# PeterFWS/Structure-PLP-SLAM

Hardware: AMD Instinct MI355X
Metric: frames/sec ORB+LSD extract+match, 640x480 TUM-RGBD, 1/2/4/8 GPU (higher is better)
Workload: dtype u8

## Files before the change

### structure-plp-slam_amd/csrc/match_kernels.hip

```cpp
#include <hip/hip_runtime.h>
#include <stdint.h>
#include <cstdlib>

#include "libstdcxx_sort.hpp"
#include "plp_barrier.hpp"
#include "match_device.hpp"
#include "plp_common.hpp"
#include "xcd_map.hpp"

namespace plp {

__device__ __forceinline__ int floor_d(double v) { int i = (int)v; return i - (i > v); }
__device__ __forceinline__ int ceil_d(double v) { int i = (int)v; return i + (i < v); }

__device__ __forceinline__ unsigned hamming256(const uint4& a0, const uint4& a1, const uint4& b0, const uint4& b1) {
    return __popc(a0.x ^ b0.x) + __popc(a0.y ^ b0.y) + __popc(a0.z ^ b0.z) + __popc(a0.w ^ b0.w) +
           __popc(a1.x ^ b1.x) + __popc(a1.y ^ b1.y) + __popc(a1.z ^ b1.z) + __popc(a1.w ^ b1.w);
}

__device__ __forceinline__ unsigned long long wave_min_u64(unsigned long long v) {
#pragma unroll
    for (int o = 32; o > 0; o >>= 1) {
        const unsigned lo = __shfl_xor((unsigned)v, o), hi = __shfl_xor((unsigned)(v >> 32), o);
        const unsigned long long w = ((unsigned long long)hi << 32) | lo;
// ... 326 lines not shown
                auto bc_f = [&](float v) -> float { return __int_as_float(__builtin_amdgcn_readlane(__float_as_int(v), u)); };
                LineTarget T;
                T.sx = bc_f(f_sx); T.sy = bc_f(f_sy); T.ex = bc_f(f_ex); T.ey = bc_f(f_ey); T.xr = bc_f(f_xr); T.xr2 = bc_f(f_xr2);
                const int misc = __builtin_amdgcn_readlane(f_misc, u);
                T.octave = misc >> 8; T.occ = (misc >> 4) & 1; T.kp_oct = (unsigned)misc & 15u;
                if (!active || !line_gate<FAM>(P, c, T, t_xr != nullptr)) continue;
                const int t = base + u;
                const uint4* d = reinterpret_cast<const uint4*>(t_desc + 32 * (size_t)t);
                const unsigned dist = hamming256(q0, q1, d[0], d[1]);
                ++passed;
                topk_insert(top, ((unsigned long long)dist << 32) | ((unsigned long long)(unsigned)t << 4) | T.kp_oct);
            }
        }
    } else if (!(c.windowed && c.empty))
        for (int t = 0; t < n; ++t) {
            const unsigned long long key = candidate_key<FAM>(P, c, t, kps, t_desc, t_xr, t_occ, q0, q1);
            if (key == ~0ull) continue;
            ++passed;
            topk_insert(top, key);
        }
    if (!active) return;
#pragma unroll
    for (int r = 0; r < kMatchK; ++r) klist[r] = pack_key(top[r]);
    *kcount = passed;
}
template <int FAM>
__global__ __launch_bounds__(64) void k_match_topk_lanes(MatchProblem P) {
    const int b = blockIdx.y;
    const int m = P.q_counts ? min(P.q_counts[b], P.m_cap) : P.m_cap;
    for (int qblock = blockIdx.x; qblock * 64 < m; qblock += gridDim.x) match_topk_lanes_block<FAM>(P, b, qblock, m);
}

constexpr int kQueriesPerBlock = 128;
constexpr int kCellStride = 4104;

__global__ __launch_bounds__(256) void k_match_prep(MatchProblem P) {
    __shared__ uint32_t cnt2[2048];
    __shared__ uint16_t start[4098];
    __shared__ uint16_t tmp_t[8192];
    __shared__ int part[4];
    const int tid = threadIdx.x, b = blockIdx.x;
    const int n = P.t_counts ? min(P.t_counts[b], P.n_cap) : P.n_cap;
    const int ncell = P.grid_cols * P.grid_rows;
    const plp_keypoint* kps = P.t_kps + (size_t)b * P.n_cap;
    const float* t_xr = P.t_x_right ? P.t_x_right + (size_t)b * P.n_cap : nullptr;
    const uint8_t* t_occ = P.t_occupied ? P.t_occupied + (size_t)b * P.n_cap : nullptr;
    StagedTarget* st = P.sorted + (size_t)b * P.n_cap;
    float* sxr = P.sorted_xr + (size_t)b * P.n_cap;
    auto cnt_inc = [&](int c) -> int { return (int)((atomicAdd(&cnt2[c >> 1], 1u << (16 * (c & 1))) >> (16 * (c & 1))) & 0xffffu); };
    for (int i = tid; i < 2048; i += 256) cnt2[i] = 0;
    wg_barrier();
    auto cell_xy = [&](float x, float y, bool occ, int& cx, int& cy) -> bool {
        cx = floor_d((double)__fsub_rn(x, P.grid_min_x) * P.inv_cell_w);
        cy = floor_d((double)__fsub_rn(y, P.grid_min_y) * P.inv_cell_h);
        return cx >= 0 && cx < P.grid_cols && cy >= 0 && cy < P.grid_rows && !occ;
    };
    for (int t0 = tid; t0 < n; t0 += 4 * 256) {
        float kx[4], ky[4]; bool oc[4];
#pragma unroll
        for (int u = 0; u < 4; ++u) { const int t = min(t0 + 256 * u, n - 1); kx[u] = kps[t].x; ky[u] = kps[t].y; oc[u] = t_occ && t_occ[t]; }
#pragma unroll
        for (int u = 0; u < 4; ++u) {
            int cx, cy;
            if (t0 + 256 * u < n && cell_xy(kx[u], ky[u], oc[u], cx, cy)) cnt_inc(cx * P.grid_rows + cy);
        }
    }
    wg_barrier();
    {
        const int lane = tid & 63, wv = tid >> 6;
        int c16[16], sum = 0;
#pragma unroll
        for (int i = 0; i < 8; ++i) { const uint32_t w = cnt2[tid * 8 + i]; c16[2 * i] = (int)(w & 0xffffu); c16[2 * i + 1] = (int)(w >> 16); sum += c16[2 * i] + c16[2 * i + 1]; }
        int inc = sum;
#pragma unroll
        for (int o = 1; o < 64; o <<= 1) { const int up = __shfl_up(inc, o); if (lane >= o) inc += up; }
        if (lane == 63) part[wv] = inc;
        wg_barrier();
        int base = inc - sum;
        for (int k = 0; k < wv; ++k) base += part[k];
#pragma unroll
        for (int i = 0; i < 16; ++i) { start[tid * 16 + i] = (uint16_t)base; base += c16[i]; }
        if (tid == 255) { start[4096] = (uint16_t)base; start[4097] = (uint16_t)base; }
        wg_barrier();
        for (int i = tid; i < 2048; i += 256) cnt2[i] = 0;
        wg_barrier();
    }
    for (int t0 = tid; t0 < n; t0 += 4 * 256) {
        float kx[4], ky[4]; bool oc[4];
#pragma unroll
        for (int u = 0; u < 4; ++u) { const int t = min(t0 + 256 * u, n - 1); kx[u] = kps[t].x; ky[u] = kps[t].y; oc[u] = t_occ && t_occ[t]; }
#pragma unroll
        for (int u = 0; u < 4; ++u) {
            const int t = t0 + 256 * u;
            int cx, cy;
            if (t >= n || !cell_xy(kx[u], ky[u], oc[u], cx, cy)) continue;
            const int cell = cx * P.grid_rows + cy;
            tmp_t[start[cell] + cnt_inc(cell)] = (uint16_t)t;
        }
    }
    wg_barrier();
    const int used = start[4096];
    for (int p0 = tid; p0 < used; p0 += 4 * 256) {
        int tt[4]; float kx[4], ky[4], xr[4] = {0.f, 0.f, 0.f, 0.f}; int ko[4];
#pragma unroll
        for (int u = 0; u < 4; ++u) {
            tt[u] = tmp_t[min(p0 + 256 * u, used - 1)];
            kx[u] = kps[tt[u]].x; ky[u] = kps[tt[u]].y; ko[u] = kps[tt[u]].octave;
            if (t_xr) xr[u] = t_xr[tt[u]];
        }
#pragma unroll
        for (int u = 0; u < 4; ++u) {
            if (p0 + 256 * u >= used) continue;
            const int t = tt[u];
            int cx, cy;
            cell_xy(kx[u], ky[u], false, cx, cy);
            const int cell = cx * P.grid_rows + cy, s0 = start[cell], s1 = start[cell + 1];
            int rank = 0;
            for (int j = s0; j < s1; ++j) rank += (int)tmp_t[j] < t;
            StagedTarget r;
            r.x = kx[u]; r.y = ky[u]; r.packed = ((uint32_t)ko[u] & 0xffu) | ((uint32_t)cx << 8) | ((uint32_t)cy << 16); r.t = (uint32_t)t;
            st[s0 + rank] = r;
            if (t_xr) sxr[s0 + rank] = xr[u];
        }
    }
    for (int i = tid; i <= ncell; i += 256) P.cell_start[(size_t)b * kCellStride + i] = start[min(i, 4096)];
}

constexpr int kLanePend = 8;
#define PLP_TOPK_CELLS_BOUNDS __launch_bounds__(256) __attribute__((amdgpu_waves_per_eu(6, 8)))

__device__ __forceinline__ uint32_t row16_min_u32(uint32_t v) {
    v = min(v, (uint32_t)__builtin_amdgcn_update_dpp((int)v, (int)v, 0x128, 0xf, 0xf, false));
    v = min(v, (uint32_t)__builtin_amdgcn_update_dpp((int)v, (int)v, 0x124, 0xf, 0xf, false));
    v = min(v, (uint32_t)__builtin_amdgcn_update_dpp((int)v, (int)v, 0x122, 0xf, 0xf, false));
    v = min(v, (uint32_t)__builtin_amdgcn_update_dpp((int)v, (int)v, 0x121, 0xf, 0xf, false));
    return v;
}
__device__ __forceinline__ int row16_sum_i32(int v) {
    v += __builtin_amdgcn_update_dpp(v, v, 0x128, 0xf, 0xf, false);
    v += __builtin_amdgcn_update_dpp(v, v, 0x124, 0xf, 0xf, false);
    v += __builtin_amdgcn_update_dpp(v, v, 0x122, 0xf, 0xf, false);
    v += __builtin_amdgcn_update_dpp(v, v, 0x121, 0xf, 0xf, false);
    return v;
}

__global__ PLP_TOPK_CELLS_BOUNDS void k_match_topk_cells(MatchProblem P, int qpb) {
    extern __shared__ __attribute__((aligned(16))) uint8_t smem[];
    unsigned uqb, ub;
    xcd_frame_major(uqb, ub);
    const int tid = threadIdx.x, b = (int)ub;
    const int m = P.q_counts ? min(P.q_counts[b], P.m_cap) : P.m_cap;
    const int q_begin = (int)uqb * qpb;
    if (q_begin >= m) return;
    const int ncell = P.grid_cols * P.grid_rows, rows = P.grid_rows;
    const uint8_t* t_desc = P.t_desc + (size_t)b * P.n_cap * 32;
    const bool has_xr = P.t_x_right != nullptr;
    const int nb = P.lds_targets;
    float2* sxy = reinterpret_cast<float2*>(smem);
    uint32_t* sto = reinterpret_cast<uint32_t*>(smem + (size_t)nb * 8);
    float* sxr = reinterpret_cast<float*>(smem + (size_t)nb * 12);
    uint16_t* cs = reinterpret_cast<uint16_t*>(smem + (size_t)nb * (has_xr ? 16 : 12));
    const uint4* g_sorted = reinterpret_cast<const uint4*>(P.sorted + (size_t)b * P.n_cap);
    const float* g_sorted_xr = P.sorted_xr + (size_t)b * P.n_cap;
    {
        const uint16_t* gcs = P.cell_start + (size_t)b * kCellStride;
        const int used = min((int)gcs[ncell], nb);
        for (int i0 = tid; i0 < used; i0 += 4 * 256) {
            uint4 r[4]; float xr[4] = {0.f, 0.f, 0.f, 0.f};
#pragma unroll
            for (int u = 0; u < 4; ++u) { const int i = min(i0 + 256 * u, used - 1); r[u] = g_sorted[i]; if (has_xr) xr[u] = g_sorted_xr[i]; }
#pragma unroll
            for (int u = 0; u < 4; ++u) {
                const int i = i0 + 256 * u;
                if (i < used) {
                    sxy[i] = make_float2(__uint_as_float(r[u].x), __uint_as_float(r[u].y));
                    sto[i] = (r[u].w & 0xffffu) | ((r[u].z & 0xffu) << 16);
                    if (has_xr) sxr[i] = xr[u];
                }
            }
        }
        const uint32_t* g32 = reinterpret_cast<const uint32_t*>(gcs);
        for (int i = tid; i < (ncell + 2) / 2; i += 256) reinterpret_cast<uint32_t*>(cs)[i] = g32[i];
    }
    __shared__ int s_dir;
    if (tid == 0) s_dir = query_direction(P, b);
    wg_barrier();
    typedef const __attribute__((address_space(3))) uint32_t* lds_u32; typedef const __attribute__((address_space(3))) float* lds_f32;
    const lds_f32 sxy_l = (lds_f32)sxy; const lds_u32 sto_l = (lds_u32)sto; const lds_f32 sxr_l = (lds_f32)sxr;
    auto t_xy = [&](int i) -> float2 { if (i < nb) return make_float2(sxy_l[2 * i], sxy_l[2 * i + 1]); const uint4 r = g_sorted[i]; return make_float2(__uint_as_float(r.x), __uint_as_float(r.y)); };
    auto t_to = [&](int i) -> uint32_t { if (i < nb) return sto_l[i]; const uint4 r = g_sorted[i]; return (r.w & 0xffffu) | ((r.z & 0xffu) << 16); };
    auto t_xr = [&](int i) -> float { return i < nb ? sxr_l[i] : g_sorted_xr[i]; };
    const uint8_t* q_valid = P.q_valid ? P.q_valid + (size_t)b * P.m_cap : nullptr;
    const int q_end = min(m, q_begin + qpb);
    static_assert(kLanePend % 2 == 0, "two positions per register");
    const int lane = tid & 63, wv = __builtin_amdgcn_readfirstlane(tid >> 6);
    for (int q_wave = q_begin + 64 * wv; q_wave < q_end; q_wave += 256) {
        const int q = q_wave + lane;
        const bool in_range = q < q_end;
        const bool active = in_range && !(q_valid && !q_valid[q]);
        uint32_t top[kMatchK], ovf[kMatchK];
#pragma unroll
        for (int i = 0; i < kMatchK; ++i) { top[i] = 0xffffffffu; ovf[i] = 0xffffffffu; }
        auto insert = [&](uint32_t key) {
            if (key < top[kMatchK - 1]) {
                const uint32_t out = top[kMatchK - 1];
                top[kMatchK - 1] = key;
#pragma unroll
                for (int e = kMatchK - 1; e > 0; --e) { const uint32_t lo = min(top[e], top[e - 1]), hi = max(top[e], top[e - 1]); top[e - 1] = lo; top[e] = hi; }
                key = out;
            }
            if (key < ovf[kMatchK - 1]) {
                ovf[kMatchK - 1] = key;
#pragma unroll
                for (int e = kMatchK - 1; e > 0; --e) { const uint32_t lo = min(ovf[e], ovf[e - 1]), hi = max(ovf[e], ovf[e - 1]); ovf[e - 1] = lo; ovf[e] = hi; }
            }
        };
        int passed = 0;
        float rx = 0.f, ry = 0.f, mg = 0.f, qxr = 0.f;
        uint32_t win = 1u, lvls = 255u << 16;
        int i = 0, i1 = 0;
        uint4 q0 = make_uint4(0u, 0u, 0u, 0u), q1 = q0;
        if (active) {
            const QueryCtx c = make_query(P, q, b, s_dir);
            if (!c.empty) {
                const uint4* qd = reinterpret_cast<const uint4*>(P.q_desc + ((size_t)b * P.q_desc_stride + q) * 32);
                q0 = qd[0]; q1 = qd[1];
                rx = c.rx; ry = c.ry; mg = c.mg; qxr = c.xr;
                win = (uint32_t)c.min_cx | ((uint32_t)c.max_cx << 8) | ((uint32_t)c.min_cy << 16) | ((uint32_t)c.max_cy << 24);
                lvls = (uint32_t)min(max(c.min_level, 0), 256) | ((c.max_level < 0 ? 255u : (uint32_t)min(c.max_level, 255)) << 16);
            }
        }
        bool wave_more;
        do {
            uint32_t pend[kLanePend / 2];
#pragma unroll
            for (int k = 0; k < kLanePend / 2; ++k) pend[k] = 0u;
            int nc = 0;
            for (;;) {
                if (i >= i1) {
                    const int col = (int)(win & 0xffu);
                    if (col <= (int)((win >> 8) & 0xffu)) {
                        i = cs[col * rows + (int)((win >> 16) & 0xffu)]; i1 = cs[col * rows + (int)(win >> 24) + 1];
                        ++win;
                    }
                } else {
                    const int p = i++;
                    const float2 sp = t_xy(p);
                    const uint32_t oct = t_to(p) >> 16;
                    bool ok = (lvls & 0xffffu) <= oct && oct <= (lvls >> 16) && fabsf(__fsub_rn(sp.x, rx)) < mg && fabsf(__fsub_rn(sp.y, ry)) < mg;
                    if (ok && has_xr) {
                        const float xr = t_xr(p);
                        ok = !(0 < xr && mg < fabsf(__fsub_rn(qxr, xr)));
                    }
                    if (ok) {
                        const uint32_t v = (uint32_t)p << (16 * (nc & 1));
#pragma unroll
                        for (int k = 0; k < kLanePend / 2; ++k) pend[k] |= (nc >> 1) == k ? v : 0u;
                        ++nc;
                    }
                }
                wave_more = __builtin_amdgcn_ballot_w64(i < i1 || (win & 0xffu) <= ((win >> 8) & 0xffu)) != 0ull;
                if (!wave_more || __builtin_amdgcn_ballot_w64(nc == kLanePend) != 0ull) break;
            }
            auto slot_pos = [&](int j) -> int { return (int)((pend[j >> 1] >> (16 * (j & 1))) & 0xffffu); };
            auto gather = [&](int j, uint4& a0, uint4& a1) {
                if (j < nc) {
                    const uint4* d = reinterpret_cast<const uint4*>(t_desc + 32 * (size_t)(t_to(slot_pos(j)) & 0xffffu));
                    a0 = d[0]; a1 = d[1];
                }
            };
            uint4 a0 = make_uint4(0u, 0u, 0u, 0u), a1 = a0;
            gather(0, a0, a1);
#pragma unroll
            for (int j = 0; j < kLanePend; ++j) {
                if (__builtin_amdgcn_ballot_w64(j < nc) == 0ull) break;
                uint4 b0 = a0, b1 = a1;
                if (j + 1 < kLanePend) gather(j + 1, b0, b1);
                if (j < nc) insert((hamming256(q0, q1, a0, a1) << 16) | (uint32_t)slot_pos(j));
                a0 = b0; a1 = b1;
            }
            passed += nc;
        } while (wave_more);
        if (!in_range) continue;
        uint32_t e[kMatchK];
#pragma unroll
        for (int k = 0; k < kMatchK; ++k) {
            e[k] = 0xffffffffu;
            if (top[k] != 0xffffffffu) {
                const uint32_t to = t_to((int)(top[k] & 0xffffu));
                e[k] = ((top[k] >> 16) << 20) | (((to >> 16) & 15u) << 16) | (to & 0xffffu);
            }
        }
        static_assert(kMatchK == 8, "two 16-byte stores per query");
        uint4* out = reinterpret_cast<uint4*>(P.klist + ((size_t)b * P.m_cap + q) * kMatchK);
        out[0] = make_uint4(e[0], e[1], e[2], e[3]);
        out[1] = make_uint4(e[4], e[5], e[6], e[7]);
        P.kcount[(size_t)b * P.m_cap + q] = active ? passed : -1;
        if (passed > kMatchK) {
#pragma unroll
            for (int k = 0; k < kMatchK; ++k) {
                e[k] = 0xffffffffu;
                if (ovf[k] != 0xffffffffu) {
                    const uint32_t to = t_to((int)(ovf[k] & 0xffffu));
                    e[k] = ((ovf[k] >> 16) << 20) | (((to >> 16) & 15u) << 16) | (to & 0xffffu);
                }
            }
            uint4* out2 = reinterpret_cast<uint4*>(P.klist2 + ((size_t)b * P.m_cap + q) * kMatchK);
            out2[0] = make_uint4(e[0], e[1], e[2], e[3]);
            out2[1] = make_uint4(e[4], e[5], e[6], e[7]);
        }
    }
}

__global__ __launch_bounds__(256) void k_match_topk_lds(MatchProblem P) {
    extern __shared__ __attribute__((aligned(16))) uint8_t smem[];
    const int tid = threadIdx.x, lane = tid & 63, wv = __builtin_amdgcn_readfirstlane(tid >> 6), b = blockIdx.y;
    const int m = P.q_counts ? min(P.q_counts[b], P.m_cap) : P.m_cap;
    const int q_begin = blockIdx.x * kQueriesPerBlock;
    if (q_begin >= m) return;
    const int n = P.t_counts ? min(P.t_counts[b], P.n_cap) : P.n_cap;
    const uint8_t* t_desc = P.t_desc + (size_t)b * P.n_cap * 32;
    uint4* sdesc = reinterpret_cast<uint4*>(smem);
    {
        const uint4* src = reinterpret_cast<const uint4*>(t_desc);
        for (int i = tid; i < 2 * n; i += 256) sdesc[i] = src[i];
    }
    wg_barrier();
    const uint8_t* q_valid = P.q_valid ? P.q_valid + (size_t)b * P.m_cap : nullptr;
    for (int q = q_begin + wv; q < min(m, q_begin + kQueriesPerBlock); q += 4) {
        uint32_t* klist = P.klist + ((size_t)b * P.m_cap + q) * kMatchK;
        int32_t* kcount = P.kcount + (size_t)b * P.m_cap + q;
        if (q_valid && !q_valid[q]) { if (lane == 0) *kcount = -1; continue; }
        const uint4* qd = reinterpret_cast<const uint4*>(P.q_desc + ((size_t)b * P.q_desc_stride + q) * 32);
        const uint4 q0 = qd[0], q1 = qd[1];
        unsigned long long top[kMatchK];
#pragma unroll
        for (int i = 0; i < kMatchK; ++i) top[i] = ~0ull;
        int passed = 0;
        for (int t = lane; t < n; t += 64) {
            const unsigned dist = hamming256(q0, q1, sdesc[2 * t], sdesc[2 * t + 1]);
            ++passed;
            topk_insert(top, ((unsigned long long)dist << 32) | ((unsigned long long)(unsigned)t << 4));
        }
#pragma unroll
        for (int o = 32; o > 0; o >>= 1) passed += __shfl_xor(passed, o);
        topk_merge_store(top, lane, klist);
        if (lane == 0) *kcount = passed;
    }
}

template <int FAM = kFamAny>
__device__ __forceinline__ bool accept(const MatchProblem& P, unsigned best, int best_lvl, unsigned second, int second_lvl) {
    const int mode = fam_mode<FAM>(P.mode);
    if (mode == PLP_MATCH_MODE_LANDMARKS || mode == PLP_MATCH_MODE_LANDMARKS_LINE) {
        if (!(best <= 100u)) return false;
        if (best_lvl == second_lvl && (float)best > __fmul_rn(P.lowe_ratio, (float)second)) return false;
        return true;
    }
    if (is_last_frame_mode(mode)) return best <= (P.hamm_dist_thr > 0 ? (unsigned)P.hamm_dist_thr : 100u);
    if (mode == PLP_MATCH_MODE_TRIANGULATION) return true;
    if (50u < best) return false;
    if (__fmul_rn(P.lowe_ratio, (float)second) < (float)best) return false;
    return true;
}

template <bool kSorted, int FAM = kFamAny>
__device__ __forceinline__ void match_resolve_body(const MatchProblem& P) {
    const int mode = fam_mode<FAM>(P.mode);
    extern __shared__ int32_t lds[];
    __shared__ int s_changed, s_num, s_hist[32], s_valid_bin[32], s_full_n, s_claim_tmp[256], s_sort_ws[48];
    __shared__ unsigned s_sort_idx[32];
    __shared__ int s_dir;
    const int tid = threadIdx.x, lane = tid & 63, wv = __builtin_amdgcn_readfirstlane(tid >> 6), b = blockIdx.x;
    const int m = P.q_counts ? min(P.q_counts[b], P.m_cap) : P.m_cap;
    const int n = P.t_counts ? min(P.t_counts[b], P.n_cap) : P.n_cap;
    int32_t* owner_final = lds;
    int32_t* owner_prev = lds + P.n_cap;
    int32_t* owner_next = lds + 2 * P.n_cap;
    const uint32_t* klist = P.klist + (size_t)b * P.m_cap * kMatchK;
    const int32_t* kcount = P.kcount + (size_t)b * P.m_cap;
    int32_t* claim = P.claim + (size_t)b * P.m_cap;
    const uint8_t* has_obs = P.q_has_obs ? P.q_has_obs + (size_t)b * P.m_cap : nullptr;
    const plp_keypoint* kps = P.t_kps ? P.t_kps + (size_t)b * P.n_cap : nullptr;
    const uint8_t* t_desc = P.t_desc + (size_t)b * P.n_cap * 32;
    const float* t_xr = P.t_x_right ? P.t_x_right + (size_t)b * P.n_cap : nullptr;
    const uint8_t* t_occ = P.t_occupied ? P.t_occupied + (size_t)b * P.n_cap : nullptr;
    int32_t* out = P.out_match + (size_t)b * P.n_cap;

    for (int t = tid; t < n; t += 256) { owner_final[t] = 0x7fffffff; out[t] = -1; }
    for (int q = tid; q < m; q += 256) claim[q] = -1;
    if (is_last_frame_mode(mode) && tid == 0) s_dir = query_direction(P, b);
    wg_barrier();

    int32_t* full_list = P.full_list + (size_t)b * P.m_cap;
    const int need = (is_last_frame_mode(mode) || mode == PLP_MATCH_MODE_TRIANGULATION) ? 1 : 2;
    const bool blocks_always = !has_obs || mode == PLP_MATCH_MODE_BRUTE_FORCE || is_group_mode(mode);
    const unsigned t_flip = mode == PLP_MATCH_MODE_TRIANGULATION ? 0xffffu : 0u;
    constexpr bool use_sorted = kSorted;
    const StagedTarget* sorted = P.sorted + (size_t)b * P.n_cap;
    const float* sorted_xr = P.sorted_xr + (size_t)b * P.n_cap;
    const uint16_t* g_cell_start = P.cell_start + (size_t)b * kCellStride;
    auto taken = [&](int t, int q, int) -> bool { return owner_final[t] != 0x7fffffff || owner_prev[t] < q; };
    {
        for (int chunk_start = 0; chunk_start < m; chunk_start += 256) {
          const int q = chunk_start + tid;
          int my_claim = -1;
          for (int t = tid; t < n; t += 256) owner_prev[t] = 0x7fffffff;
          constexpr int kList = kSorted ? 2 * kMatchK : kMatchK;
          uint32_t e8[kList];
          int cnt = 0;
          if (q < m) {
              cnt = kcount[q];
              const uint4* kp = reinterpret_cast<const uint4*>(klist + (size_t)q * kMatchK);
              const uint4 lo = kp[0], hi = kp[1];
              e8[0] = lo.x; e8[1] = lo.y; e8[2] = lo.z; e8[3] = lo.w; e8[4] = hi.x; e8[5] = hi.y; e8[6] = hi.z; e8[7] = hi.w;
              if constexpr (kSorted) {
#pragma unroll
                  for (int k = kMatchK; k < kList; ++k) e8[k] = 0xffffffffu;
                  if (cnt > kMatchK) {
                      const uint4* kp2 = reinterpret_cast<const uint4*>(P.klist2 + ((size_t)b * P.m_cap + q) * kMatchK);
                      const uint4 lo2 = kp2[0], hi2 = kp2[1];
                      e8[8] = lo2.x; e8[9] = lo2.y; e8[10] = lo2.z; e8[11] = lo2.w; e8[12] = hi2.x; e8[13] = hi2.y; e8[14] = hi2.z; e8[15] = hi2.w;
                  }
              }
          }
          for (int inner = 0; inner <= 256; ++inner) {
            if (tid == 0) { s_full_n = 0; s_changed = 0; }
            for (int t = tid; t < n; t += 256) owner_next[t] = 0x7fffffff;
            wg_barrier();
            int new_claim = -1;
            bool decided = false;
            if (q < m) {
                if (cnt <= 0) decided = true;
                else {
                    const int have = min(cnt, kList);
                    unsigned best = 256, second = 256;
                    int best_lvl = -1, second_lvl = -1, best_t = -1, found = 0;
#pragma unroll
                    for (int e = 0; e < kList; ++e) {
                        if (e >= have || found >= need) continue;
                        const int t = (int)((e8[e] & 0xffff) ^ t_flip);
                        if (taken(t, q, chunk_start)) continue;
                        if (found == 0) { best = e8[e] >> 20; best_lvl = (int)((e8[e] >> 16) & 15); best_t = t; }
                        else { second = e8[e] >> 20; second_lvl = (int)((e8[e] >> 16) & 15); }
                        ++found;
                    }
                    bool rescan = found < need && cnt > kList;
                    if (rescan && mode != PLP_MATCH_MODE_TRIANGULATION) {
                        const unsigned d8 = e8[kList - 1] >> 20;
                        const bool lm = mode == PLP_MATCH_MODE_LANDMARKS || mode == PLP_MATCH_MODE_LANDMARKS_LINE;
                        const unsigned thr = (lm || is_last_frame_mode(mode)) ? (is_last_frame_mode(mode) && P.hamm_dist_thr > 0 ? (unsigned)P.hamm_dist_thr : 100u) : 50u;
                        if (found == 0) { if (d8 > thr) rescan = false; }
                        else if (best > thr) rescan = false;
                        else if (lm) { if (!((float)best > __fmul_rn(P.lowe_ratio, (float)d8))) { rescan = false; second = d8; second_lvl = -2; } }
                        else if (!(__fmul_rn(P.lowe_ratio, (float)d8) < (float)best)) { rescan = false; second = d8; }
                    }
                    if (rescan) full_list[atomicAdd(&s_full_n, 1)] = q;
                    else { decided = true; if (found > 0 && accept<FAM>(P, best, best_lvl, second, second_lvl)) new_claim = best_t; }
                }
            }
            wg_barrier();
            const int nf = s_full_n;
            if (tid == 0 && P.dbg && nf) atomicAdd(&P.dbg[0], nf);
            for (int f = wv; f < nf; f += 4) {
                const int fq = full_list[f];
                const QueryCtx c = make_query<FAM>(P, fq, b, s_dir);
                const uint4* qd = reinterpret_cast<const uint4*>(P.q_desc + ((size_t)b * P.q_desc_stride + fq) * 32);
                const uint4 q0 = qd[0], q1 = qd[1];
                unsigned long long k0 = ~0ull, k1 = ~0ull;
                if constexpr (use_sorted) {
                    if (!c.empty) {
                        const bool check_level = (0 < c.min_level) || (0 <= c.max_level);
                        for (int col = c.min_cx; col <= c.max_cx; ++col) {
                            const int i0 = g_cell_start[col * P.grid_rows + c.min_cy], i1 = g_cell_start[col * P.grid_rows + c.max_cy + 1];
                            for (int i = i0 + lane; i < i1; i += 64) {
                                const StagedTarget s = sorted[i];
                                const int oct = (int)(s.packed & 0xff);
                                if (check_level) {
                                    if (oct < c.min_level) continue;
                                    if (0 <= c.max_level && c.max_level < oct) continue;
                                }
                                if (!(fabsf(__fsub_rn(s.x, c.rx)) < c.mg && fabsf(__fsub_rn(s.y, c.ry)) < c.mg)) continue;
                                if (t_xr) {
                                    const float xr = sorted_xr[i];
                                    if (0 < xr && c.mg < fabsf(__fsub_rn(c.xr, xr))) continue;
                                }
                                if (taken((int)s.t, fq, chunk_start)) continue;
                                const uint4* d = reinterpret_cast<const uint4*>(t_desc + 32 * (size_t)s.t);
                                const unsigned dist = hamming256(q0, q1, d[0], d[1]);
                                const unsigned long long key = ((unsigned long long)dist << 32) | ((unsigned long long)(unsigned)i << 4) | (unsigned)(oct & 15);
                                if (key < k0) { k1 = k0; k0 = key; } else if (key < k1) k1 = key;
                            }
                        }
                    }
                } else if (!(c.windowed && c.empty)) {
                    for (int t = lane; t < n; t += 64) {
                        if (taken(t, fq, chunk_start)) continue;
                        const unsigned long long key = candidate_key<FAM>(P, c, t, kps, t_desc, t_xr, t_occ, q0, q1);
                        if (key < k0) { k1 = k0; k0 = key; } else if (key < k1) k1 = key;
                    }
                }
                const unsigned long long g0 = wave_min_u64(k0);
                const unsigned long long g1 = wave_min_u64(k0 == g0 ? k1 : k0);
                if (lane == 0) {
                    int nc = -1;
                    if (g0 != ~0ull) {
                        const unsigned second = g1 != ~0ull ? (unsigned)(g1 >> 32) : 256u;
                        const int second_lvl = g1 != ~0ull ? (int)(g1 & 15) : -1;
                        if (accept<FAM>(P, (unsigned)(g0 >> 32), (int)(g0 & 15), second, second_lvl))
                            nc = use_sorted ? (int)sorted[(g0 >> 4) & 0xffff].t : (int)(((g0 >> 4) & 0xffff) ^ t_flip);
                    }
                    s_claim_tmp[fq - chunk_start] = nc;
                }
            }
            wg_barrier();
            if (q < m) {
                if (!decided) new_claim = s_claim_tmp[tid];
                if (my_claim != new_claim) { my_claim = new_claim; s_changed = 1; }
                if (new_claim >= 0 && (blocks_always || has_obs[q])) atomicMin(&owner_next[new_claim], q);
            }
            wg_barrier();
            { int32_t* t = owner_prev; owner_prev = owner_next; owner_next = t; }
            const int changed = s_changed;
            wg_barrier();
            if (!changed) break;
          }
          if (tid == 0 && P.dbg) atomicAdd(&P.dbg[1], 1);
          if (q < m) {
              claim[q] = my_claim;
              if (my_claim >= 0 && (blocks_always || has_obs[q])) atomicMin(&owner_final[my_claim], q);
          }
          wg_barrier();
        }
    }

    if (tid == 0) s_num = 0;
    for (int i = tid; i < 32; i += 256) { s_hist[i] = 0; s_valid_bin[i] = 0; }
    wg_barrier();
    const bool angle_check = P.check_orientation && (mode == PLP_MATCH_MODE_LAST_FRAME || mode == PLP_MATCH_MODE_BRUTE_FORCE || is_group_mode(mode));
    const float* q_angle = P.q_angle ? P.q_angle + (size_t)b * P.m_cap : nullptr;
    const float* t_angle = P.t_angle ? P.t_angle + (size_t)b * P.n_cap : nullptr;
    auto bin_of = [&](int q, int t) -> int {
        const float ta = kps ? kps[t].angle : t_angle[t];
        float delta = (mode == PLP_MATCH_MODE_LAST_FRAME || is_group_mode(mode)) ? __fsub_rn(q_angle[q], ta) : __fsub_rn(ta, q_angle[q]);
        if (delta < 0.0) delta = (float)((double)delta + 360.0);
        if (360.0 <= delta) delta = (float)((double)delta - 360.0);
        const int bin = __float2int_rn(__fmul_rn(delta, 1.0f / 30));
        return (unsigned)bin > 31u ? 31 : bin;
    };
    int my = 0;
    for (int q = tid; q < m; q += 256) {
        const int t = claim[q];
        if (t < 0) continue;
        ++my;
        atomicMax(&out[t], q);
        if (angle_check) atomicAdd(&s_hist[min(bin_of(q, t), 31)], 1);
    }
    if (my) atomicAdd(&s_num, my);
    wg_barrier();
    if (angle_check) {
        if (tid == 0) {
            libstdcxx::index_sort_by_size(s_hist, 30, s_sort_idx, s_sort_ws);
            for (int r = 0; r < 3; ++r) s_valid_bin[s_sort_idx[r]] = 1;
        }
        wg_barrier();
        int bad = 0;
        for (int q = tid; q < m; q += 256) {
            const int t = claim[q];
            if (t < 0) continue;
            if (!s_valid_bin[min(bin_of(q, t), 31)]) { out[t] = (P.flags & PLP_MATCH_FLAG_MARK_INVALIDATED) ? -2 : -1; ++bad; }
        }
        if (bad) atomicSub(&s_num, bad);
        wg_barrier();
    }
    if (tid == 0) P.out_num[b] = s_num;
}
__global__ __launch_bounds__(256) __attribute__((amdgpu_waves_per_eu(4, 8))) void k_match_resolve_sorted(MatchProblem P) { match_resolve_body<true, kFamGrid>(P); }
template <int FAM>
__global__ __launch_bounds__(256) void k_match_resolve_generic(MatchProblem P) { match_resolve_body<false, FAM>(P); }

__global__ __launch_bounds__(256) void k_hamming_matrix(const uint8_t* __restrict__ qd, int nq, const uint8_t* __restrict__ td, int nt,
                                                        uint16_t* __restrict__ dist) {
    __shared__ uint32_t sq[64 * 9], st[64 * 9];
    const int tid = threadIdx.x;
    const int q0 = blockIdx.y * 64, t0 = blockIdx.x * 64;
    for (int i = tid; i < 64 * 8; i += 256) {
        const int r = i >> 3, w = i & 7;
        sq[r * 9 + w] = q0 + r < nq ? reinterpret_cast<const uint32_t*>(qd)[(size_t)(q0 + r) * 8 + w] : 0u;
        st[r * 9 + w] = t0 + r < nt ? reinterpret_cast<const uint32_t*>(td)[(size_t)(t0 + r) * 8 + w] : 0u;
    }
    wg_barrier();
    const int tx = tid & 63, ty = __builtin_amdgcn_readfirstlane(tid >> 6);
    uint32_t tv[8];
#pragma unroll
    for (int w = 0; w < 8; ++w) tv[w] = st[tx * 9 + w];
    for (int r = ty; r < 64; r += 4) {
        unsigned d = 0;
#pragma unroll
        for (int w = 0; w < 8; ++w) d += __popc(sq[r * 9 + w] ^ tv[w]);
        if (q0 + r < nq && t0 + tx < nt) dist[(size_t)(q0 + r) * nt + t0 + tx] = (uint16_t)d;
    }
}

__global__ __launch_bounds__(256) void k_match_fuse(MatchProblem P) {
    const int lane = threadIdx.x & 63, b = blockIdx.y;
    const int q = blockIdx.x * 4 + __builtin_amdgcn_readfirstlane((int)(threadIdx.x >> 6));
    const int m = P.q_counts ? min(P.q_counts[b], P.m_cap) : P.m_cap;
    if (q >= m) return;
    int32_t* out = P.out_query_best + (size_t)b * P.m_cap + q;
    const uint8_t* q_valid = P.q_valid ? P.q_valid + (size_t)b * P.m_cap : nullptr;
    if (q_valid && !q_valid[q]) { if (lane == 0) *out = -1; return; }
    const int n = P.t_counts ? min(P.t_counts[b], P.n_cap) : P.n_cap;
    const plp_keypoint* kps = P.t_kps + (size_t)b * P.n_cap;
    const uint8_t* t_desc = P.t_desc + (size_t)b * P.n_cap * 32;
    const float* t_xr = P.t_x_right ? P.t_x_right + (size_t)b * P.n_cap : nullptr;
    const QueryCtx c = make_query(P, q, b, query_direction(P, b));
    const uint4* qd = reinterpret_cast<const uint4*>(P.q_desc + ((size_t)b * P.q_desc_stride + q) * 32);
    const uint4 q0 = qd[0], q1 = qd[1];
    unsigned long long best = ~0ull;
    if (!c.empty)
        for (int t = lane; t < n; t += 64) {
            const unsigned long long key = candidate_key(P, c, t, kps, t_desc, t_xr, nullptr, q0, q1);
            best = key < best ? key : best;
        }
    best = wave_min_u64(best);
    const unsigned thr = P.hamm_dist_thr > 0 ? (unsigned)P.hamm_dist_thr : 50u;
    if (lane == 0) *out = (best != ~0ull && (unsigned)(best >> 32) <= thr) ? (int32_t)((best >> 4) & 0xffff) : -1;
}

__global__ __launch_bounds__(64) void k_match_area(AreaArgs A) {
    __shared__ int hist[32], valid_bin[32], sort_ws[48];
    __shared__ unsigned sort_idx[32];
    const int lane = threadIdx.x;
    uint32_t* mdist = A.scratch;
    int32_t* m1in2 = reinterpret_cast<int32_t*>(A.scratch + A.n2);
    for (int i = lane; i < A.n2; i += 64) { mdist[i] = 256u; m1in2[i] = -1; }
    for (int i = lane; i < A.n1; i += 64) A.matched_2_in_1[i] = -1;
    if (lane < 32) { hist[lane] = 0; valid_bin[lane] = 0; }
    __builtin_amdgcn_fence(__ATOMIC_ACQ_REL, "workgroup");
    __builtin_amdgcn_wave_barrier();
    auto bin_of = [&](int i1, int i2) -> int {
        float delta = __fsub_rn(A.kps1[i1].angle, A.kps2[i2].angle);
        if (delta < 0.0) delta = (float)((double)delta + 360.0);
        if (360.0 <= delta) delta = (float)((double)delta - 360.0);
        const int bin = __float2int_rn(__fmul_rn(delta, 1.0f / 30));
        return (unsigned)bin > 31u ? 31 : bin;
    };
    for (int i1 = 0; i1 < A.n1; ++i1) {
        const plp_keypoint k1 = A.kps1[i1];
        if (0 < k1.octave) continue;
        const float rx = A.prev_pts[2 * i1], ry = A.prev_pts[2 * i1 + 1], mg = A.margin;
        const int min_cx = max(0, floor_d((double)__fsub_rn(__fsub_rn(rx, A.grid_min_x), mg) * A.inv_cell_w));
        const int max_cx = min(A.grid_cols - 1, ceil_d((double)__fadd_rn(__fsub_rn(rx, A.grid_min_x), mg) * A.inv_cell_w));
        const int min_cy = max(0, floor_d((double)__fsub_rn(__fsub_rn(ry, A.grid_min_y), mg) * A.inv_cell_h));
        const int max_cy = min(A.grid_rows - 1, ceil_d((double)__fadd_rn(__fsub_rn(ry, A.grid_min_y), mg) * A.inv_cell_h));
        if (A.grid_cols <= min_cx || max_cx < 0 || A.grid_rows <= min_cy || max_cy < 0) continue;
        const uint4* qd = reinterpret_cast<const uint4*>(A.desc1 + 32 * (size_t)i1);
        const uint4 q0 = qd[0], q1 = qd[1];
        unsigned long long k0 = ~0ull, k1k = ~0ull;
        for (int t = lane; t < A.n2; t += 64) {
            const plp_keypoint k = A.kps2[t];
            const int cx = floor_d((double)__fsub_rn(k.x, A.grid_min_x) * A.inv_cell_w), cy = floor_d((double)__fsub_rn(k.y, A.grid_min_y) * A.inv_cell_h);
            if (cx < 0 || cx >= A.grid_cols || cy < 0 || cy >= A.grid_rows) continue;
            if (cx < min_cx || cx > max_cx || cy < min_cy || cy > max_cy) continue;
            if (k.octave < 0 || 0 < k.octave) continue;
            if (!(fabsf(__fsub_rn(k.x, rx)) < mg && fabsf(__fsub_rn(k.y, ry)) < mg)) continue;
            const uint4* d = reinterpret_cast<const uint4*>(A.desc2 + 32 * (size_t)t);
            const unsigned dist = hamming256(q0, q1, d[0], d[1]);
            if (mdist[t] <= dist) continue;
            const unsigned long long key = ((unsigned long long)dist << 32) | ((unsigned long long)(((unsigned)(cx * A.grid_rows + cy) << 16) | (unsigned)t));
            if (key < k0) { k1k = k0; k0 = key; } else if (key < k1k) k1k = key;
        }
        const unsigned long long g0 = wave_min_u64(k0);
        const unsigned long long g1 = wave_min_u64(k0 == g0 ? k1k : k0);
        if (g0 == ~0ull) continue;
        const unsigned best = (unsigned)(g0 >> 32), second = g1 != ~0ull ? (unsigned)(g1 >> 32) : 256u;
        if (50u < best) continue;
        if (__fmul_rn((float)second, A.lowe_ratio) < (float)best) continue;
        const int best_i2 = (int)(g0 & 0xffff);
        if (lane == 0) {
            const int prev_i1 = m1in2[best_i2];
            if (0 <= prev_i1) A.matched_2_in_1[prev_i1] = -1;
            A.matched_2_in_1[i1] = best_i2;
            m1in2[best_i2] = i1;
            mdist[best_i2] = best;
            if (A.check_orientation) hist[bin_of(i1, best_i2)] += 1;
        }
        __builtin_amdgcn_fence(__ATOMIC_ACQ_REL, "workgroup");
        __builtin_amdgcn_wave_barrier();
    }
    if (A.check_orientation && lane == 0) {
        libstdcxx::index_sort_by_size(hist, 30, sort_idx, sort_ws);
        for (int r = 0; r < 3; ++r) valid_bin[sort_idx[r]] = 1;
    }
    __builtin_amdgcn_fence(__ATOMIC_ACQ_REL, "workgroup");
    __builtin_amdgcn_wave_barrier();
    int cnt = 0;
    for (int i1 = lane; i1 < A.n1; i1 += 64) {
        const int i2 = A.matched_2_in_1[i1];
        if (i2 < 0) continue;
        if (A.check_orientation && !valid_bin[bin_of(i1, i2)]) { A.matched_2_in_1[i1] = -1; continue; }
        ++cnt;
        A.prev_pts[2 * i1] = A.kps2[i2].x; A.prev_pts[2 * i1 + 1] = A.kps2[i2].y;
    }
#pragma unroll
    for (int o = 32; o > 0; o >>= 1) cnt += __shfl_xor(cnt, o);
    if (lane == 0) *A.num_matches = cnt;
}

void launch_match_area(hipStream_t st, const AreaArgs& A) { hipLaunchKernelGGL(k_match_area, dim3(1), dim3(64), 0, st, A); }

static bool is_line_mode_host(int mode) { return mode == PLP_MATCH_MODE_LANDMARKS_LINE || mode == PLP_MATCH_MODE_LAST_FRAME_LINE || mode == PLP_MATCH_MODE_FUSE_LINE; }

MatchPlan plan_match(const MatchProblem& P, int B) {
    MatchPlan pl{kTopkNone, kFamAny, 0, kResolveNone, 0};
    if (P.mode == PLP_MATCH_MODE_FUSE || P.mode == PLP_MATCH_MODE_FUSE_LINE) { pl.topk = kTopkFuse; return pl; }
    const bool windowed = P.mode == PLP_MATCH_MODE_LANDMARKS || P.mode == PLP_MATCH_MODE_LAST_FRAME;
    const bool line = is_line_mode_host(P.mode) || P.mode == PLP_MATCH_MODE_BOW || P.mode == PLP_MATCH_MODE_TRIANGULATION;
    pl.family = is_line_mode_host(P.mode) ? kFamLine : (P.mode == PLP_MATCH_MODE_BOW || P.mode == PLP_MATCH_MODE_TRIANGULATION) ? kFamGroup : kFamPoint;
    pl.staged = windowed ? (size_t)P.lds_targets * (P.t_x_right ? 16 : 12) + 2 * kCellStride : (size_t)P.n_cap * 32;
    pl.resolve = kResolveGeneric;
// ... 102 lines not shown
```

Baseline: 97820.

## Compact live queries and replace owner arrays with generation-keyed round map in resolve

In the top-k kernel, a workgroup whose queries are all invalid now writes kcount=-1 and exits before staging targets into LDS. In the resolve kernel, queries with a positive candidate count are compacted per wave into a live list with ballot/mbcnt, and the iterative claim rounds run only over that list. The per-round owner_prev/owner_next arrays, which had to be reset every round, are replaced by a double-buffered round_map keyed by generation and priority via atomicMax, so the resets and one barrier per round go away. Rescan queries are tracked in an LDS byte list. The risks are subtle changes to claim-ordering semantics and the extra compaction pass.

```diff
diff --git a/structure-plp-slam_amd/csrc/match_kernels.hip b/structure-plp-slam_amd/csrc/match_kernels.hip
--- a/structure-plp-slam_amd/csrc/match_kernels.hip
+++ b/structure-plp-slam_amd/csrc/match_kernels.hip
@@ -502,6 +502,20 @@
     const int m = P.q_counts ? min(P.q_counts[b], P.m_cap) : P.m_cap;
     const int q_begin = (int)uqb * qpb;
     if (q_begin >= m) return;
+    const uint8_t* q_valid = P.q_valid ? P.q_valid + (size_t)b * P.m_cap : nullptr;
+    const int q_end = min(m, q_begin + qpb);
+    if (q_valid) {
+        __shared__ int s_wave_live[4];
+        bool live = false;
+        for (int q = q_begin + tid; q < q_end; q += 256) live = live || q_valid[q] != 0;
+        const bool wave_live = __builtin_amdgcn_ballot_w64(live) != 0ull;
+        if ((tid & 63) == 0) s_wave_live[tid >> 6] = wave_live;
+        wg_barrier();
+        if (!(s_wave_live[0] | s_wave_live[1] | s_wave_live[2] | s_wave_live[3])) {
+            for (int q = q_begin + tid; q < q_end; q += 256) P.kcount[(size_t)b * P.m_cap + q] = -1;
+            return;
+        }
+    }
     const int ncell = P.grid_cols * P.grid_rows, rows = P.grid_rows;
     const uint8_t* t_desc = P.t_desc + (size_t)b * P.n_cap * 32;
     const bool has_xr = P.t_x_right != nullptr;
@@ -540,8 +554,6 @@
     auto t_xy = [&](int i) -> float2 { if (i < nb) return make_float2(sxy_l[2 * i], sxy_l[2 * i + 1]); const uint4 r = g_sorted[i]; return make_float2(__uint_as_float(r.x), __uint_as_float(r.y)); };
     auto t_to = [&](int i) -> uint32_t { if (i < nb) return sto_l[i]; const uint4 r = g_sorted[i]; return (r.w & 0xffffu) | ((r.z & 0xffu) << 16); };
     auto t_xr = [&](int i) -> float { return i < nb ? sxr_l[i] : g_sorted_xr[i]; };
-    const uint8_t* q_valid = P.q_valid ? P.q_valid + (size_t)b * P.m_cap : nullptr;
-    const int q_end = min(m, q_begin + qpb);
     static_assert(kLanePend % 2 == 0, "two positions per register");
     const int lane = tid & 63, wv = __builtin_amdgcn_readfirstlane(tid >> 6);
     for (int q_wave = q_begin + 64 * wv; q_wave < q_end; q_wave += 256) {
@@ -718,15 +730,15 @@
 __device__ __forceinline__ void match_resolve_body(const MatchProblem& P) {
     const int mode = fam_mode<FAM>(P.mode);
     extern __shared__ int32_t lds[];
-    __shared__ int s_changed, s_num, s_hist[32], s_valid_bin[32], s_full_n, s_claim_tmp[256], s_sort_ws[48];
-    __shared__ unsigned s_sort_idx[32];
+    __shared__ int s_num, s_hist[32], s_valid_bin[32], s_full_n[2], s_claim_tmp[256], s_sort_ws[48], s_wave_live[4];
+    __shared__ unsigned s_sort_idx[32], s_changed[2];
+    __shared__ uint8_t s_full[256];
     __shared__ int s_dir;
     const int tid = threadIdx.x, lane = tid & 63, wv = __builtin_amdgcn_readfirstlane(tid >> 6), b = blockIdx.x;
     const int m = P.q_counts ? min(P.q_counts[b], P.m_cap) : P.m_cap;
     const int n = P.t_counts ? min(P.t_counts[b], P.n_cap) : P.n_cap;
     int32_t* owner_final = lds;
-    int32_t* owner_prev = lds + P.n_cap;
-    int32_t* owner_next = lds + 2 * P.n_cap;
+    uint32_t* round_map = reinterpret_cast<uint32_t*>(lds) + P.n_cap;
     const uint32_t* klist = P.klist + (size_t)b * P.m_cap * kMatchK;
     const int32_t* kcount = P.kcount + (size_t)b * P.m_cap;
     int32_t* claim = P.claim + (size_t)b * P.m_cap;
@@ -737,12 +749,35 @@
     const uint8_t* t_occ = P.t_occupied ? P.t_occupied + (size_t)b * P.n_cap : nullptr;
     int32_t* out = P.out_match + (size_t)b * P.n_cap;
 
-    for (int t = tid; t < n; t += 256) { owner_final[t] = 0x7fffffff; out[t] = -1; }
-    for (int q = tid; q < m; q += 256) claim[q] = -1;
+    for (int t = tid; t < n; t += 256) { owner_final[t] = 0x7fffffff; round_map[t] = 0u; round_map[P.n_cap + t] = 0u; out[t] = -1; }
+    if (tid < 2) { s_changed[tid] = 0u; s_full_n[tid] = 0; }
     if (is_last_frame_mode(mode) && tid == 0) s_dir = query_direction(P, b);
-    wg_barrier();
-
-    int32_t* full_list = P.full_list + (size_t)b * P.m_cap;
+    int32_t* live_list = P.full_list + (size_t)b * P.m_cap;
+    const int seg = (m + 255) / 256 * 64, seg_begin = wv * seg, seg_end = min(m, seg_begin + seg);
+    {
+        int at = seg_begin;
+        for (int q0 = seg_begin + lane; q0 < seg_end + lane; q0 += 256) {
+            int c[4];
+#pragma unroll
+            for (int u = 0; u < 4; ++u) c[u] = q0 + 64 * u < seg_end ? kcount[q0 + 64 * u] : 0;
+#pragma unroll
+            for (int u = 0; u < 4; ++u) {
+                const int q = q0 + 64 * u;
+                const unsigned long long mask = __builtin_amdgcn_ballot_w64(c[u] > 0);
+                if (q < seg_end) claim[q] = -1;
+                if (c[u] > 0) live_list[at + (int)__builtin_amdgcn_mbcnt_hi((unsigned)(mask >> 32), __builtin_amdgcn_mbcnt_lo((unsigned)mask, 0u))] = q;
+                at += __popcll(mask);
+            }
+        }
+        if (lane == 0) s_wave_live[wv] = at - seg_begin;
+    }
+    wg_barrier_after_global_stores();
+    int n_live = s_wave_live[0] + s_wave_live[1] + s_wave_live[2] + s_wave_live[3];
+    auto live_at = [&](int r) -> int {
+        const int c0 = s_wave_live[0], c1 = s_wave_live[1], c2 = s_wave_live[2];
+        return live_list[r + (r >= c0 ? seg - c0 : 0) + (r >= c0 + c1 ? seg - c1 : 0) + (r >= c0 + c1 + c2 ? seg - c2 : 0)];
+    };
+
     const int need = (is_last_frame_mode(mode) || mode == PLP_MATCH_MODE_TRIANGULATION) ? 1 : 2;
     const bool blocks_always = !has_obs || mode == PLP_MATCH_MODE_BRUTE_FORCE || is_group_mode(mode);
     const unsigned t_flip = mode == PLP_MATCH_MODE_TRIANGULATION ? 0xffffu : 0u;
@@ -750,16 +785,21 @@
     const StagedTarget* sorted = P.sorted + (size_t)b * P.n_cap;
     const float* sorted_xr = P.sorted_xr + (size_t)b * P.n_cap;
     const uint16_t* g_cell_start = P.cell_start + (size_t)b * kCellStride;
-    auto taken = [&](int t, int q, int) -> bool { return owner_final[t] != 0x7fffffff || owner_prev[t] < q; };
+    unsigned gen = 1u;
+    n_live = __builtin_amdgcn_readfirstlane(n_live);
+    auto taken = [&](int t, unsigned my_key) -> bool { return (owner_final[t] != 0x7fffffff) | (round_map[(gen & 1u) * (unsigned)P.n_cap + t] > my_key); };
     {
-        for (int chunk_start = 0; chunk_start < m; chunk_start += 256) {
-          const int q = chunk_start + tid;
+        int q_next = tid < n_live ? live_at(tid) : -1;
+        for (int chunk_start = 0; chunk_start < n_live; chunk_start += 256) {
+          const int q = q_next;
+          q_next = chunk_start + 256 + tid < n_live ? live_at(chunk_start + 256 + tid) : -1;
           int my_claim = -1;
-          for (int t = tid; t < n; t += 256) owner_prev[t] = 0x7fffffff;
           constexpr int kList = kSorted ? 2 * kMatchK : kMatchK;
           uint32_t e8[kList];
           int cnt = 0;
-          if (q < m) {
+          unsigned blocks = 0u;
+          if (q >= 0) {
+              if (blocks_always || has_obs[q]) blocks = 256u - (unsigned)tid;
               cnt = kcount[q];
               const uint4* kp = reinterpret_cast<const uint4*>(klist + (size_t)q * kMatchK);
               const uint4 lo = kp[0], hi = kp[1];
@@ -774,23 +814,32 @@
                   }
               }
           }
-          for (int inner = 0; inner <= 256; ++inner) {
-            if (tid == 0) { s_full_n = 0; s_changed = 0; }
-            for (int t = tid; t < n; t += 256) owner_next[t] = 0x7fffffff;
-            wg_barrier();
+          for (int inner = 0; inner <= 256; ++inner, ++gen) {
+            const unsigned slot = gen & 1u, my_key = (gen << 8) | (255u - (unsigned)tid);
+            uint32_t* map_w = round_map + (slot ^ 1u) * (unsigned)P.n_cap;
             int new_claim = -1;
-            bool decided = false;
-            if (q < m) {
-                if (cnt <= 0) decided = true;
-                else {
+#pragma unroll
+            for (int e = 0; e < kList; ++e) asm volatile("" : "+v"(e8[e]));
+            asm volatile("" : "+v"(cnt));
+            if (q >= 0) {
+                {
                     const int have = min(cnt, kList);
                     unsigned best = 256, second = 256;
                     int best_lvl = -1, second_lvl = -1, best_t = -1, found = 0;
+                    unsigned taken_bits = 0u;
+#pragma unroll
+                    for (int e = 0; e < kMatchK; ++e) taken_bits |= (unsigned)taken(e < have ? (int)((e8[e] & 0xffff) ^ t_flip) : 0, my_key) << e;
+                    if constexpr (kList > kMatchK) {
+                        if (have > kMatchK) {
+#pragma unroll
+                            for (int e = kMatchK; e < kList; ++e) taken_bits |= (unsigned)taken(e < have ? (int)((e8[e] & 0xffff) ^ t_flip) : 0, my_key) << e;
+                        }
+                    }
 #pragma unroll
                     for (int e = 0; e < kList; ++e) {
                         if (e >= have || found >= need) continue;
                         const int t = (int)((e8[e] & 0xffff) ^ t_flip);
-                        if (taken(t, q, chunk_start)) continue;
+                        if ((taken_bits >> e) & 1u) continue;
                         if (found == 0) { best = e8[e] >> 20; best_lvl = (int)((e8[e] >> 16) & 15); best_t = t; }
                         else { second = e8[e] >> 20; second_lvl = (int)((e8[e] >> 16) & 15); }
                         ++found;
@@ -805,15 +854,23 @@
                         else if (lm) { if (!((float)best > __fmul_rn(P.lowe_ratio, (float)d8))) { rescan = false; second = d8; second_lvl = -2; } }
                         else if (!(__fmul_rn(P.lowe_ratio, (float)d8) < (float)best)) { rescan = false; second = d8; }
                     }
-                    if (rescan) full_list[atomicAdd(&s_full_n, 1)] = q;
-                    else { decided = true; if (found > 0 && accept<FAM>(P, best, best_lvl, second, second_lvl)) new_claim = best_t; }
+                    if (rescan) { s_full[atomicAdd(&s_full_n[slot], 1)] = (uint8_t)tid; new_claim = -2; }
+                    else if (found > 0 && accept<FAM>(P, best, best_lvl, second, second_lvl)) new_claim = best_t;
                 }
             }
+            auto settle = [&](int nc) {
+                if (my_claim != nc) { my_claim = nc; s_changed[slot] = gen; }
+                if (nc >= 0 && blocks) atomicMax(&map_w[nc], ((gen + 1u) << 8) + blocks - 1u);
+            };
+            if (new_claim != -2) settle(new_claim);
             wg_barrier();
-            const int nf = s_full_n;
-            if (tid == 0 && P.dbg && nf) atomicAdd(&P.dbg[0], nf);
+            const int nf = __builtin_amdgcn_readfirstlane(s_full_n[slot]);
+            if (nf) {
+            if (tid == 0 && P.dbg) atomicAdd(&P.dbg[0], nf);
             for (int f = wv; f < nf; f += 4) {
-                const int fq = full_list[f];
+                const int f_local = s_full[f];
+                const unsigned f_key = (gen << 8) | (255u - (unsigned)f_local);
+                const int fq = live_at(chunk_start + f_local);
                 const QueryCtx c = make_query<FAM>(P, fq, b, s_dir);
                 const uint4* qd = reinterpret_cast<const uint4*>(P.q_desc + ((size_t)b * P.q_desc_stride + fq) * 32);
                 const uint4 q0 = qd[0], q1 = qd[1];
@@ -835,7 +892,7 @@
                                     const float xr = sorted_xr[i];
                                     if (0 < xr && c.mg < fabsf(__fsub_rn(c.xr, xr))) continue;
                                 }
-                                if (taken((int)s.t, fq, chunk_start)) continue;
+                                if (taken((int)s.t, f_key)) continue;
                                 const uint4* d = reinterpret_cast<const uint4*>(t_desc + 32 * (size_t)s.t);
                                 const unsigned dist = hamming256(q0, q1, d[0], d[1]);
                                 const unsigned long long key = ((unsigned long long)dist << 32) | ((unsigned long long)(unsigned)i << 4) | (unsigned)(oct & 15);
@@ -845,7 +902,7 @@
                     }
                 } else if (!(c.windowed && c.empty)) {
                     for (int t = lane; t < n; t += 64) {
-                        if (taken(t, fq, chunk_start)) continue;
+                        if (taken(t, f_key)) continue;
                         const unsigned long long key = candidate_key<FAM>(P, c, t, kps, t_desc, t_xr, t_occ, q0, q1);
                         if (key < k0) { k1 = k0; k0 = key; } else if (key < k1) k1 = key;
                     }
@@ -860,25 +917,21 @@
                         if (accept<FAM>(P, (unsigned)(g0 >> 32), (int)(g0 & 15), second, second_lvl))
                             nc = use_sorted ? (int)sorted[(g0 >> 4) & 0xffff].t : (int)(((g0 >> 4) & 0xffff) ^ t_flip);
                     }
-                    s_claim_tmp[fq - chunk_start] = nc;
+                    s_claim_tmp[f_local] = nc;
                 }
             }
             wg_barrier();
-            if (q < m) {
-                if (!decided) new_claim = s_claim_tmp[tid];
-                if (my_claim != new_claim) { my_claim = new_claim; s_changed = 1; }
-                if (new_claim >= 0 && (blocks_always || has_obs[q])) atomicMin(&owner_next[new_claim], q);
-            }
+            if (tid == 0) s_full_n[slot] = 0;
+            if (new_claim == -2) settle(s_claim_tmp[tid]);
             wg_barrier();
-            { int32_t* t = owner_prev; owner_prev = owner_next; owner_next = t; }
-            const int changed = s_changed;
-            wg_barrier();
-            if (!changed) break;
+            }
+            if (__builtin_amdgcn_readfirstlane(s_changed[slot]) != gen) break;
           }
+          gen += 2u;
           if (tid == 0 && P.dbg) atomicAdd(&P.dbg[1], 1);
-          if (q < m) {
+          if (q >= 0) {
               claim[q] = my_claim;
-              if (my_claim >= 0 && (blocks_always || has_obs[q])) atomicMin(&owner_final[my_claim], q);
+              if (my_claim >= 0 && blocks) atomicMin(&owner_final[my_claim], q);
           }
           wg_barrier();
         }
@@ -899,8 +952,8 @@
         return (unsigned)bin > 31u ? 31 : bin;
     };
     int my = 0;
-    for (int q = tid; q < m; q += 256) {
-        const int t = claim[q];
+    for (int i = tid; i < n_live; i += 256) {
+        const int q = live_at(i), t = claim[q];
         if (t < 0) continue;
         ++my;
         atomicMax(&out[t], q);
@@ -915,8 +968,8 @@
         }
         wg_barrier();
         int bad = 0;
-        for (int q = tid; q < m; q += 256) {
-            const int t = claim[q];
+        for (int i = tid; i < n_live; i += 256) {
+            const int q = live_at(i), t = claim[q];
             if (t < 0) continue;
             if (!s_valid_bin[min(bin_of(q, t), 31)]) { out[t] = (P.flags & PLP_MATCH_FLAG_MARK_INVALIDATED) ? -2 : -1; ++bad; }
         }
```

Result: no change. 98710, median of 6 (+0.9%).
